# viniciusvidal2/slam-sensor-fusion

Hardware: AMD Instinct MI355X
Metric: scans_per_s_200k_scan_vs_10M_map (higher is better)
Workload: dtype f32 points / f64 accumulation

## Files before the change

### include/slamfusion.h

```cpp
#ifndef SLAMFUSION_H
#define SLAMFUSION_H
#include <stdint.h>

#ifdef __cplusplus
extern "C" {
#endif

#define SF_VERSION 210

typedef enum {
    SF_OK = 0,
    SF_ERR_INVALID = -1,
    SF_ERR_HIP = -2,
    SF_ERR_NOMEM = -3,
    SF_ERR_STATE = -4,
    SF_ERR_OVERFLOW = -5,
    SF_ERR_COMM = -6
} sf_status;

typedef struct sf_ctx sf_ctx;
typedef struct sf_cloud sf_cloud;
typedef struct sf_map sf_map;
typedef struct sf_icp sf_icp;

// ... 178 lines not shown
int sf_icp_fused_count(sf_icp *icp, int64_t *launches);
int sf_icp_fused_redone(sf_icp *icp, int64_t *redone);
int sf_icp_test_inject_barrier_timeout(sf_icp *icp);
#define SF_ORDER_AUTO 0
#define SF_ORDER_AS_GIVEN 1
#define SF_ORDER_CELL 2
int sf_icp_set_query_order(sf_icp *icp, int order);
int sf_icp_set_nn_reuse(sf_icp *icp, int on);
int sf_icp_set_wide_scan_points(sf_icp *icp, int64_t points);
int sf_icp_set_pipeline(sf_icp *icp, int on);
int sf_icp_set_tile_search(sf_icp *icp, int mode);
int sf_icp_tile_info(sf_icp *icp, int64_t out[12]);
int sf_icp_set_freeze(sf_icp *icp, int on);
int sf_icp_set_freeze_params(sf_icp *icp, float guard_scale, float guard_min, float guard_max, int max_tries, int from_launch);
int sf_icp_freeze_stats(sf_icp *icp, int64_t out[5]);
int sf_icp_set_defer_search(sf_icp *icp, int on);
int sf_icp_defer_stats(sf_icp *icp, int64_t out[2]);
int sf_icp_lookup_launch_stats(sf_icp *icp, int64_t out[4]);
int sf_icp_set_neighbour_research(sf_icp *icp, int from_launch);
int sf_icp_neighbour_stats(sf_icp *icp, int64_t out[3]);
int sf_icp_neighbour_gap_stats(sf_icp *icp, int64_t out[4]);
#define SF_ROBUST_NONE 0
#define SF_ROBUST_HUBER 1
#define SF_ROBUST_CAUCHY 2
#define SF_ROBUST_TUKEY 3
#define SF_ROBUST_GM 4
int sf_icp_set_robust_kernel(sf_icp *icp, int kind, double k);

#define SF_COV_EIG_EPS 1e-12
#define SF_COV_FEW_CORR 1
// ... 201 lines not shown
#define SF_TEST_OP_ROBUST 7
#define SF_TEST_OP_EIGVEC 8
int sf_test_linalg(sf_ctx *ctx, int op, const double *in, int in_stride, int64_t cases, double *out, int out_stride);
int sf_test_wave_reduce(sf_ctx *ctx, int width , const double *in , double *out );
int sf_test_block_reduce(sf_ctx *ctx, int nrec , const double *in , double *out );
int sf_test_reduce_partials(sf_ctx *ctx, int nrec , int nt , const double *part , int nblocks, double *out );

int sf_test_plane_score(sf_cloud *c, const float *planes, int64_t n_planes, double t, int max_blocks, int64_t *counts);

int sf_test_label_boxes(sf_cloud *c, const int32_t *labels, int64_t n_labels, const sf_box_params *p, int max_blocks,
                        sf_label_box *boxes, sf_box_stats *stats);

#define SF_TEST_SCHEDULE_IN 15
#define SF_TEST_SCHEDULE_OUT 10
int sf_test_launch_schedule(const int32_t *in, int64_t rows, int k, int32_t *out);

#ifdef __cplusplus
}
#endif
#endif
```

### slam_sensor_fusion_amd/api.py

```python
import atexit
import ctypes as C
import math
import os
import weakref

import numpy as np

_HERE = os.path.dirname(os.path.abspath(__file__))
LIB_PATH = os.path.join(_HERE, "lib", "libslamfusion.so")

SF_ICP_REF_CPP, SF_ICP_O3D_P2P, SF_ICP_P2PLANE = 0, 1, 2
SF_VOXEL_PCL, SF_VOXEL_O3D, SF_VOXEL_PCL64 = 0, 1, 2
SF_FLAG_VOXEL_OVERFLOW = 1
SF_ICP_FLAG_FEW_CORR, SF_ICP_FLAG_SINGULAR, SF_ICP_FLAG_SHARD_STALE, SF_ICP_FLAG_BARRIER_TIMEOUT = 1, 2, 4, 8
PROF_NN, PROF_REDUCE, PROF_COLLECTIVE, PROF_SOLVE, PROF_SHARD_BUILD = 0, 1, 2, 3, 4
SF_ERR_COMM = -6
MODES = {"ref_cpp": SF_ICP_REF_CPP, "o3d_p2p": SF_ICP_O3D_P2P, "p2plane": SF_ICP_P2PLANE}
ROBUST_KINDS = {"none": 0, "huber": 1, "cauchy": 2, "tukey": 3, "gm": 4}


class SlamFusionError(RuntimeError):
    pass


# ... 166 lines not shown
    lib.sf_test_linalg.argtypes = [C.c_void_p, C.c_int, C.c_void_p, C.c_int, C.c_int64, C.c_void_p, C.c_int]
    lib.sf_test_wave_reduce.argtypes = [C.c_void_p, C.c_int, C.c_void_p, C.c_void_p]
    lib.sf_test_block_reduce.argtypes = [C.c_void_p, C.c_int, C.c_void_p, C.c_void_p]
    lib.sf_test_reduce_partials.argtypes = [C.c_void_p, C.c_int, C.c_int, C.c_void_p, C.c_int, C.c_void_p]
    lib.sf_plane_default_params.restype = None
    lib.sf_cloud_plane_hypotheses.argtypes = [C.c_void_p, C.c_void_p, C.c_void_p, C.c_void_p, C.c_void_p]
    lib.sf_cloud_score_planes.argtypes = [C.c_void_p, C.c_void_p, C.c_int64, C.c_double, C.c_void_p]
    lib.sf_cloud_segment_plane.argtypes = [C.c_void_p, C.c_void_p, C.c_void_p, C.c_void_p, C.c_void_p]
    lib.sf_cloud_remove_plane.argtypes = [C.c_void_p, C.c_void_p, C.c_int, C.c_void_p, C.c_void_p]
    lib.sf_test_plane_score.argtypes = [C.c_void_p, C.c_void_p, C.c_int64, C.c_double, C.c_int, C.c_void_p]
    lib.sf_cloud_label_boxes.argtypes = [C.c_void_p, C.c_void_p, C.c_int64, C.c_void_p, C.c_void_p, C.c_void_p]
    lib.sf_test_label_boxes.argtypes = [C.c_void_p, C.c_void_p, C.c_int64, C.c_void_p, C.c_int, C.c_void_p, C.c_void_p]
    lib.sf_cloud_cluster_boxes.argtypes = [C.c_void_p, C.c_double, C.c_int64, C.c_int64, C.c_float, C.c_void_p, C.c_void_p, C.c_int64, C.c_void_p, C.c_void_p]
    lib.sf_cloud_remove_boxes.argtypes = [C.c_void_p, C.c_void_p, C.c_void_p, C.c_void_p, C.c_int64, C.c_double, C.c_int, C.c_void_p]
    lib.sf_test_launch_schedule.argtypes = [C.c_void_p, C.c_int64, C.c_int, C.c_void_p]
    _lib = lib
    return lib


def voxel_merge_min_points(n=-1):
    return int(load_library().sf_cloud_voxel_merge_min_points(C.c_int64(n)))


def kernel_source_hash():
    import hashlib
    h = hashlib.sha256()
    for name in ("sf_icp.hip", "sf_nn_red_body.inc", "sf_nn.hpp", "sf_tile.hpp", "sf_order.hpp", "sf_common.hpp", "sf_schedule.hpp"):
        with open(os.path.join(_HERE, "csrc", name), "rb") as f:
            h.update(f.read())
    return h.hexdigest()[:16]
# ... 14 lines not shown

def _p(a):
    return a.ctypes.data_as(C.c_void_p)


SCHEDULE_INPUTS = ("mode", "K", "qpl", "sharded", "whole", "reuse", "window", "robust", "wanted", "fz_from", "defer", "table", "nbr_from", "lk_min", "tile_on")
SCHEDULE_OUTPUTS = ("launches", "nn", "one_per_lane", "solve_takes_freeze_state", "ask_freeze", "deferred_rows", "attempt_from", "fz", "lookup_first", "defer_first")
NN_SEARCH, NN_TILE_SEARCH, NN_DEFERRING, NN_FREEZE, NN_FROZEN_FEW = range(5)


def hook_launch_schedule(configs, k):
    configs = np.ascontiguousarray(configs, dtype=np.int32).reshape(-1, len(SCHEDULE_INPUTS))
    out = np.empty((len(configs), len(SCHEDULE_OUTPUTS)), np.int32)
    _check(load_library().sf_test_launch_schedule(_p(configs), len(configs), int(k), _p(out)))
    return out


def hook_plane_score(cloud, planes, distance_threshold, max_blocks=0):
    planes = _f32(planes).reshape(-1, 4)
    counts = np.empty(len(planes), np.int64)
    _check(cloud.lib.sf_test_plane_score(cloud.h, _p(planes), len(planes), float(distance_threshold), int(max_blocks), _p(counts)))
    return counts


def hook_label_boxes(cloud, labels, n_labels=None, mode="pca", up=None, max_blocks=0):
    return cloud._label_boxes(labels, n_labels, mode, up, False, int(max_blocks))


def hook_radix_sort(ctx, keys, vals, end_bit, lead=0, lead_alt=0):
    keys = np.ascontiguousarray(keys)
# ... 698 lines not shown
        _check(self.lib.sf_icp_set_tile_search(self.h, C.c_int(code)))

    def tile_info(self):
        a = (C.c_int64 * 12)()
        _check(self.lib.sf_icp_tile_info(self.h, a))
        return {"on": bool(a[0]), "cells_per_tile": [a[1], a[2], a[3]], "tiles": [a[4], a[5], a[6]], "searched": a[7], "from_lds": a[8], "left_region": a[9],
                "beyond_ring_1": a[10], "tiles_too_dense": a[11]}

    def set_freeze_params(self, guard_scale=8.0, guard_min=2.0e-5, guard_max=3.0e-4, max_tries=3, from_launch=5):
        _check(self.lib.sf_icp_set_freeze_params(self.h, C.c_float(guard_scale), C.c_float(guard_min), C.c_float(guard_max), C.c_int(max_tries), C.c_int(from_launch)))

    def freeze_stats(self):
        a = (C.c_int64 * 5)()
        _check(self.lib.sf_icp_freeze_stats(self.h, a))
        return {"froze": a[0], "thawed": a[1], "failed": a[2], "active_queries": a[3], "frozen_at_end": a[4]}

    def set_defer_search(self, on=True):
        _check(self.lib.sf_icp_set_defer_search(self.h, C.c_int(int(bool(on)))))

    def set_neighbour_research(self, from_launch=2):
        _check(self.lib.sf_icp_set_neighbour_research(self.h, C.c_int(int(from_launch))))

    def neighbour_stats(self):
        a = (C.c_int64 * 3)()
        _check(self.lib.sf_icp_neighbour_stats(self.h, a))
        return {"served": a[0], "not_served": a[1], "waves_searched": a[2]}

    def neighbour_gap_stats(self):
        a = (C.c_int64 * 4)()
        _check(self.lib.sf_icp_neighbour_gap_stats(self.h, a))
# ... 674 lines not shown
```

### slam_sensor_fusion_amd/csrc/sf_icp.hip

```cpp
#include "sf_common.hpp"
#include "sf_nn.hpp"
#include "sf_tile.hpp"
#include "sf_order.hpp"
#include "sf_p2p.hpp"
#include "sf_schedule.hpp"

#include <cfloat>
#include <cstdlib>
#include <cmath>
#include <vector>
#include <mutex>
#include <string>

namespace {

constexpr int BLK = 256;
constexpr int NREC_P2P = 17;
constexpr int NREC_PLANE = 30;
constexpr int REC_STRIDE = 32;

struct IcpState {
    double T[16];
    double rec[REC_STRIDE];
    double fitness, rmse, prev_fitness, prev_rmse;
    float last_error, err_pending;
    float step[12];
    int step_pending;
    int iterations, done, research, n_corr, n_research, flags, converged;
    int n_points;
    int cache_live;
    int froze_launch;
    double T_list[12];
    double motion;
};

struct IcpParams {
    float max_corr;
    float accept;
    float eps;
    int num_iters;
};

inline unsigned nblk(int64_t n, int b = 256) { return (unsigned)sf::div_up(n > 0 ? n : 1, b); }

__device__ __forceinline__ void mat4_mul(const double A[16], const double B[16], double C[16])
{
    double R[16];
#pragma unroll
// ... 329 lines not shown
    int b = blockIdx.x * blockDim.x + threadIdx.x;
    if (b >= batch) return;
    IcpState s;
    for (int i = 0; i < 16; ++i) s.T[i] = inits ? inits[16 * b + i] : args.T[b][i];
    for (int i = 0; i < REC_STRIDE; ++i) s.rec[i] = 0;
    s.fitness = s.rmse = s.prev_fitness = s.prev_rmse = 0;
    s.last_error = FLT_MAX;
    s.err_pending = 0;
    for (int i = 0; i < 12; ++i) s.step[i] = 0;
    s.step_pending = 0;
    s.iterations = s.done = s.research = s.n_corr = s.n_research = s.flags = s.converged = 0;
    s.n_points = -1;
    s.cache_live = 0;
    s.froze_launch = -1;
    s.motion = 0.0;
    for (int i = 0; i < 12; ++i) s.T_list[i] = s.T[i];
    st[b] = s;
}

constexpr int64_t WIDE_SCAN_POINTS = 131072;
constexpr int64_t WIDE_AUTO_POINTS = 65536;
using sf::VERIFY_FROM_SEARCH;
#ifndef NN_RED_WAVES
#define NN_RED_WAVES 4
#endif
#ifndef SF_NBR_FROM
#define SF_NBR_FROM 2
#endif
constexpr int NN_STATS_SHARDS = 256;
constexpr int NN_STATS_PER = 5;
// ... 871 lines not shown

__device__ __forceinline__ void track_motion(IcpState *S, const double *To, const ScanBox &box)
{
    double worst = 0.0;
    for (int c = 0; c < 8; ++c) {
        const double x = (c & 1) ? box.hi[0] : box.lo[0], y = (c & 2) ? box.hi[1] : box.lo[1], z = (c & 4) ? box.hi[2] : box.lo[2];
        double d2 = 0.0;
        for (int r = 0; r < 3; ++r) {
            const double d = (S->T[4 * r] - To[4 * r]) * x + (S->T[4 * r + 1] - To[4 * r + 1]) * y + (S->T[4 * r + 2] - To[4 * r + 2]) * z + (S->T[4 * r + 3] - To[4 * r + 3]);
            d2 += d * d;
        }
        worst = d2 > worst ? d2 : worst;
    }
    const double step = sqrt(worst) * 1.000001 + 1.0e-9;
    S->motion = (step == step) ? S->motion + step : 1.0e30;
    S->cache_live = 1;
}

__device__ __forceinline__ void solve_o3d(IcpState *S, const double *rec, int n_src, int k, int K)
{
    k = S->n_research;
    const double n = rec[0];
    const double fitness = n_src > 0 ? n / (double)n_src : 0.0;
    const double rmse = n > 0 ? sqrt(rec[16] / n) : 0.0;
    S->fitness = fitness;
    S->rmse = rmse;
    S->n_corr = (int)n;
    S->n_research += 1;
    if (k > 0 && fabs(S->prev_fitness - fitness) < 1e-6 && fabs(S->prev_rmse - rmse) < 1e-6) {
        S->converged = 1;
// ... 76 lines not shown
constexpr int FZ_NMOM = 96;
constexpr int FZ_CAP = 128;
constexpr int64_t FREEZE_AUTO_MIN_QUERIES = 700000;
struct FreezeState {
    int mode;
    int tries;
    int froze, thawed;
    int64_t n_active;
    float guard;
    int launch_mode;
    double motion0;
    double Tf[12];
    double D[12];
    double mom[FZ_NMOM];
};
struct FreezeParams { float guard_scale, guard_min, guard_max; int max_tries; };

__device__ __forceinline__ constexpr int k6a(int k) { return k < 3 ? 0 : (k < 5 ? 1 : 2); }
__device__ __forceinline__ constexpr int k6b(int k) { return k < 3 ? k : (k < 5 ? k - 2 : 2); }
__device__ __forceinline__ constexpr int k6(int a, int b) { return a <= b ? (a == 0 ? b : (a == 1 ? 2 + b : 5)) : (b == 0 ? a : (b == 1 ? 2 + a : 5)); }

struct MomIn { double x[3], n[3], p[3], c, w; };
__device__ __forceinline__ MomIn mom_in(const LanePair &P, bool take)
{
    MomIn t;
    const bool ok = P.ok && take;
    t.w = ok ? 1.0 : 0.0;
    t.x[0] = ok ? P.sx : 0.0; t.x[1] = ok ? P.sy : 0.0; t.x[2] = ok ? P.sz : 0.0;
    t.p[0] = (double)(ok ? P.px : 0.0f); t.p[1] = (double)(ok ? P.py : 0.0f); t.p[2] = (double)(ok ? P.pz : 0.0f);
    t.n[0] = (double)(ok ? P.tn.x : 0.0f); t.n[1] = (double)(ok ? P.tn.y : 0.0f); t.n[2] = (double)(ok ? P.tn.z : 0.0f);
    t.c = t.n[0] * t.p[0] + t.n[1] * t.p[1] + t.n[2] * t.p[2];
// ... 654 lines not shown
                F->mode = 0;
                F->tries += 1;
            } else {
                F->mode = 2;
                F->froze += 1;
                if (S->froze_launch < 0) S->froze_launch = S->n_research;
                F->motion0 = S->motion;
                for (int i = 0; i < 12; ++i) { F->Tf[i] = S->T[i]; F->D[i] = (i % 5 == 0) ? 1.0 : 0.0; }
                for (int i = 0; i < FZ_NMOM; ++i) F->mom[i] = mom[i];
            }
        }
    }
    __syncthreads();
}

__device__ __forceinline__ void freeze_after_update(const IcpState *S, FreezeState *F, double m0, double m1, const FreezeParams &fp, int request, const double *upd)
{
    if (F->mode == 2) {
        double Dn[12];
        for (int r = 0; r < 3; ++r) {
            for (int c = 0; c < 4; ++c) Dn[4 * r + c] = upd[4 * r] * F->D[c] + upd[4 * r + 1] * F->D[4 + c] + upd[4 * r + 2] * F->D[8 + c] + (c == 3 ? upd[4 * r + 3] : 0.0);
        }
        for (int i = 0; i < 12; ++i) F->D[i] = Dn[i];
    }
    if (F->mode == 2 && !(m1 - F->motion0 <= (double)F->guard * 0.98)) {
        F->mode = 0;
        F->tries += 1;
        F->thawed += 1;
    }
    if (F->mode == 0 && F->launch_mode == 0 && request && !S->done && F->tries < fp.max_tries) {
        const float gd = fmaxf((float)(m1 - m0) * fp.guard_scale, fp.guard_min);
        if (gd <= fp.guard_max) { F->guard = gd; F->mode = 1; }
    }
}

__global__ __launch_bounds__(RBLK) void k_reduce_solve_fz(IcpState *__restrict__ st, const double *__restrict__ partials, int nblocks, int n_src, int K,
                                                          const ScanBox *__restrict__ boxp, FreezeBufs fb, FreezeParams fp, int request)
{
    const int b = blockIdx.x;
    IcpState *S = st + b;
    if (S->done) return;
    FreezeState *F = fb.fz + b;
    __shared__ double rec[REC_STRIDE];
    freeze_fold<RBLK>(S, F, b, partials, nblocks, nblocks, fb, rec);
    if (fb.df_part) add_deferred_rows(fb.df_part, b, rec);
    if (threadIdx.x == 0) {
        for (int c = 0; c < NREC_PLANE; ++c) S->rec[c] = rec[c];
        double To[12];
// ... 579 lines not shown
    int64_t fused_redone = 0;
    bool inject_timeout = false;
    int64_t fused_launches = 0;
    IcpState *h_pin = nullptr;
    size_t h_pin_cap = 0;
    bool use_graph = false;
    int64_t graph_captures = 0, graph_replays = 0;
    struct GraphKey {
        int batch = -1, ordered = -1, robust_kind = -1, cov_on = -1;
        sf::Schedule sched;
        int64_t n = -1;
        const void *map = nullptr;
        uint64_t map_generation = 0, epochs = 0;
        uint64_t nbr_stamp = 0;
        const void *nbr = nullptr;
        float max_corr = 0, accept = 0, eps = 0, guard_scale = 0, guard_min = 0, guard_max = 0;
        int max_tries = 0;
        double robust_k = 0;
        double cov_prm[5] = {0, 0, 0, 0, 0};
        bool operator==(const GraphKey &o) const
        {
            return batch == o.batch && ordered == o.ordered && sched == o.sched && n == o.n && map == o.map && map_generation == o.map_generation && epochs == o.epochs &&
                   nbr_stamp == o.nbr_stamp && nbr == o.nbr && max_corr == o.max_corr && accept == o.accept && eps == o.eps &&
                   guard_scale == o.guard_scale && guard_min == o.guard_min && guard_max == o.guard_max && max_tries == o.max_tries &&
                   robust_kind == o.robust_kind && robust_k == o.robust_k && cov_on == o.cov_on && std::memcmp(cov_prm, o.cov_prm, sizeof(cov_prm)) == 0;
        }
    };
    struct LaneMeta {
        bool valid = false;
        bool cov = false;
        int batch = 0, mode = 0;
        std::vector<double> inits;
        int src_set = 0;
        uint64_t src_version = 0;
        sf::Schedule sched;
        int64_t lk_waves = 0;
    };
    struct Lane {
        sf::DevBuf X;
// ... 55 lines not shown
    bool unfetched = false;
    bool mark_valid = false;
    uint64_t src_version = 0, mark_src_version = 0, mark_map_generation = 0;
    const void *mark_map = nullptr;
    SfWindow mark_window{};
    bool profiling = false;
    std::vector<hipEvent_t> ev;
    size_t ev_used = 0;
    int64_t prof_launches = 0;
    double prof_ms = 0;
    std::vector<float> prof_each;
    std::vector<int> ev_kind;
    std::vector<float> prof_phase[SF_PROF_KINDS];
    sf::DevBuf nn_stats;
    int freeze = 1;
    FreezeParams fz_prm{8.0f, 2.0e-5f, 3.0e-4f, 3};
    int fz_from = 5;
    bool fz_from_auto = true;
    int fz_fetches = 0;
    int fz_step = 0;
    int nbr_from = SF_NBR_FROM;
    bool nbr_active = false;
    int64_t nbr_stats_first = 0;
    uint64_t mark_nbr_stamp = 0;
    int defer = 1;
    int lk_min = 0;
    int64_t nn_stats_used = 0;
    static constexpr int64_t NN_STATS_CAP = 1024;
    int robust_kind = SF_ROBUST_NONE;
    double robust_k = 0.0;
    int cov_on = 0;
    CovArg cov_arg{0.0, 0.0, 0.0, 0.0, 0.0};
    bool prev_cov_ok = false;
    int tile_mode = 0;
// ... 392 lines not shown
}

sf_icp::GraphKey graph_key_now(const sf_icp *icp, int mode)
{
    const Lane &ln = icp->cur(); const SrcSet &ss = icp->src();
    sf_icp::GraphKey k;
    k.batch = ss.batch; k.ordered = (int)icp->ordered; k.sched = ln.meta.sched;
    k.n = (mode == SF_ICP_REF_CPP && ss.batch == 1) ? -ss.n_cap : ss.n;
    k.map = (const void *)icp->map;
    k.map_generation = icp->map->generation;
    if (icp->nbr_active) { k.nbr_stamp = icp->map->nbr_stamp; k.nbr = icp->map->nbr.p; }
    k.robust_kind = robust_on(icp, mode) ? icp->robust_kind : SF_ROBUST_NONE; k.robust_k = robust_on(icp, mode) ? icp->robust_k : 0.0;
    k.cov_on = icp->cov_on;
    if (icp->cov_on) { const double cp[5] = {icp->cov_arg.sensor_sigma, icp->cov_arg.thr_t, icp->cov_arg.thr_r, icp->cov_arg.infl_t, icp->cov_arg.infl_r}; std::memcpy(k.cov_prm, cp, sizeof(cp)); }
    k.max_corr = icp->prm.max_corr; k.accept = icp->prm.accept; k.eps = icp->prm.eps;
    k.guard_scale = icp->fz_prm.guard_scale; k.guard_min = icp->fz_prm.guard_min; k.guard_max = icp->fz_prm.guard_max; k.max_tries = icp->fz_prm.max_tries;
    const sf::DevBuf *bufs[] = {&ss.X0, &ss.X0r, &ln.X, &ln.Xq, &ln.qcache, &ln.corr, &ln.state, &ln.partials, &icp->d_box, &ss.d_boxes, &ss.n_dev,
                                &icp->map->pts4, &icp->map->nrm4, &icp->map->cell_start, &icp->map->d_window, &ln.fz_state, &ln.fz_part, &ln.fz_cnt, &ln.fz_ids, &ln.fz_all, &ln.df_cnt, &ln.df_ids, &ln.df_part, &ln.df_stat, &ln.tseg, &ln.tile_stats, &ln.cov_part, &ln.cov_out};
    k.epochs = (uint64_t)ss.plane;
    for (const sf::DevBuf *b : bufs) k.epochs = (k.epochs * 1000003ull + b->epoch) * 1000003ull + (uint64_t)(uintptr_t)b->p;
    return k;
}

SfGrid grid_for(const sf_icp *icp)
{
    SfGrid g = icp->map->grid;
    g.nbr = icp->nbr_active ? icp->map->nbr.as<uint4>() : nullptr;
    g.nbr_from = icp->nbr_from;
    return g;
}

// ... 841 lines not shown
    out[1] = df[0];
    out[2] = df[1];
    out[3] = sched.lookup_first;
    return SF_OK;
}

extern "C" int sf_icp_set_freeze(sf_icp *icp, int on)
{
    SF_CHECK(icp, SF_ERR_INVALID, "icp is NULL");
    SF_CHECK(on >= 0 && on <= 2, SF_ERR_INVALID, "sf_icp_set_freeze: 0 (off), 1 (auto) or 2 (always)");
    icp->freeze = on;
    return SF_OK;
}

namespace {
constexpr int FZ_FROM_DEFAULT = 5, FZ_PROBE_EVERY = 32;
void freeze_learn_schedule(sf_icp *icp)
{
    const sf::Schedule &sched = icp->cur().meta.sched;
    if (!icp->fz_from_auto || icp->last_fused || icp->shard || icp->last_mode != SF_ICP_P2PLANE) return;
    const int K = sched.K;
    if (++icp->fz_fetches >= FZ_PROBE_EVERY) { icp->fz_fetches = 0; icp->fz_from = FZ_FROM_DEFAULT; icp->lk_min = 0; return; }
    if (!sched.fz) return;
    if (sched.lookup_launches() > 0 && icp->cur().df_stat.p) {
        uint32_t h[2 + DF_STAT_LAUNCHES];
        if (hipMemcpy(h, icp->cur().df_stat.p, sizeof(h), hipMemcpyDeviceToHost) == hipSuccess) {
            for (int k = sched.lookup_first; k < sched.fz_from && k < DF_STAT_LAUNCHES - 1; ++k)
                if ((int64_t)h[2 + k] * 8 > icp->cur().meta.lk_waves) icp->lk_min = std::max(icp->lk_min, k + 1);
        }
    }
    int latest = -1, never = 0;
    for (int b = 0; b < icp->src().batch; ++b) {
        const IcpState &S = icp->h_state[(size_t)b];
        if (S.froze_launch >= 0) latest = std::max(latest, S.froze_launch);
        else if (S.iterations >= K) never += 1;
    }
    if (latest < 0) icp->fz_from = std::max(FZ_FROM_DEFAULT, K);
    else if (never * 4 <= icp->src().batch) icp->fz_from = std::min(std::max(FZ_FROM_DEFAULT, latest), std::max(FZ_FROM_DEFAULT, K - 2));
}
}

extern "C" int sf_icp_set_robust_kernel(sf_icp *icp, int kind, double k)
{
    SF_CHECK(icp, SF_ERR_INVALID, "icp is NULL");
    SF_CHECK(kind >= SF_ROBUST_NONE && kind <= SF_ROBUST_GM, SF_ERR_INVALID, "unknown robust kernel %d", kind);
    SF_CHECK(kind == SF_ROBUST_NONE || (std::isfinite(k) && k > 0.0), SF_ERR_INVALID, "the robust kernel's scale must be finite and > 0 (got %g)", k);
    icp->robust_kind = kind;
    icp->robust_k = kind == SF_ROBUST_NONE ? 0.0 : k;
    return SF_OK;
}

extern "C" int sf_icp_set_freeze_params(sf_icp *icp, float guard_scale, float guard_min, float guard_max, int max_tries, int from_launch)
{
    SF_CHECK(icp, SF_ERR_INVALID, "icp is NULL");
    SF_CHECK(guard_scale >= 0.0f && guard_min >= 0.0f && guard_max >= guard_min && max_tries >= 0 && from_launch >= VERIFY_FROM_SEARCH && from_launch < 1024, SF_ERR_INVALID,
             "bad freeze parameters");
    icp->fz_prm = FreezeParams{guard_scale, guard_min, guard_max, max_tries};
    icp->fz_from = from_launch;
    icp->fz_from_auto = false;
    icp->lk_min = 0;
    return SF_OK;
}

extern "C" int sf_icp_freeze_stats(sf_icp *icp, int64_t out[5])
{
    SF_CHECK(icp && out, SF_ERR_INVALID, "bad arguments");
    Lane &ln = icp->cur(); SrcSet &ss = icp->src();
    for (int i = 0; i < 5; ++i) out[i] = 0;
    const int nb = ln.meta.valid && ln.meta.batch > 0 && !icp->shard ? ln.meta.batch : ss.batch;
    if (!ln.meta.sched.fz || icp->last_fused || !ln.fz_state.p || nb <= 0) return SF_OK;
    std::vector<FreezeState> h((size_t)nb);
    SF_HIP(hipMemcpyAsync(h.data(), ln.fz_state.p, sizeof(FreezeState) * h.size(), hipMemcpyDeviceToHost, icp->ctx->stream));
    SF_HIP(hipStreamSynchronize(icp->ctx->stream));
    for (const FreezeState &f : h) {
        out[0] += f.froze;
        out[1] += f.thawed;
        out[2] += f.tries - f.thawed;
        out[3] += f.n_active;
        out[4] += f.mode == 2 ? 1 : 0;
    }
    return SF_OK;
}

extern "C" int sf_icp_graph_counts(sf_icp *icp, int64_t *captures, int64_t *launches)
{
    SF_CHECK(icp, SF_ERR_INVALID, "icp is NULL");
    if (captures) *captures = icp->graph_captures;
    if (launches) *launches = icp->graph_replays;
    return SF_OK;
}

extern "C" int sf_icp_set_fused(sf_icp *icp, int on)
{
    SF_CHECK(icp, SF_ERR_INVALID, "icp is NULL");
    icp->fused = on != 0;
// ... 236 lines not shown

extern "C" int sf_icp_fetch_results(sf_icp *icp, sf_icp_result *out)
{
    SF_CHECK(icp && out, SF_ERR_INVALID, "bad arguments");
    const Lane &ln = icp->cur(); const SrcSet &ss = icp->src();
    SF_CHECK(ss.batch > 0, SF_ERR_STATE, "nothing to fetch");
    const bool described = ln.meta.valid && ln.meta.batch > 0 && !icp->shard;
    const int nb = described ? ln.meta.batch : ss.batch;
    SF_TRY(states_to_host(icp, nb));
    icp->unfetched = false;
    fused_release(icp);
    if (icp->profiling) prof_collect(icp);
    SF_TRY(check_barrier_flags(icp, nb));
    for (int b = 0; b < nb; ++b)
        fill_result(icp, described ? ln.meta.mode : icp->last_mode, icp->h_state[(size_t)b], described ? &ln.meta.inits[(size_t)b * 16] : &icp->inits[(size_t)b * 16], out + b);
    if (nb == ss.batch) freeze_learn_schedule(icp);
    return SF_OK;
}

extern "C" int sf_icp_fetch_previous(sf_icp *icp, sf_icp_result *out)
{
    SF_CHECK(icp && out, SF_ERR_INVALID, "bad arguments");
    Lane &pl = icp->prev();
    const sf_icp::LaneMeta &M = pl.meta;
    SF_CHECK(icp->prev_ok && M.valid && M.batch > 0, SF_ERR_STATE,
             "no earlier alignment to fetch: the latest alignment did not run beside the one before it (fetched in between, pipeline off, single launch) or it was fetched already");
    SF_CHECK(pl.used && pl.done && pl.stream && pl.state.p, SF_ERR_STATE, "the other lane holds no alignment");
    SF_HIP(hipSetDevice(icp->ctx->device));
    SF_HIP(hipEventSynchronize(pl.done));
    icp->h_prev.resize((size_t)M.batch);
    SF_HIP(hipMemcpyAsync(icp->h_prev.data(), pl.state.p, sizeof(IcpState) * (size_t)M.batch, hipMemcpyDeviceToHost, pl.stream));
    SF_HIP(hipStreamSynchronize(pl.stream));
    for (int b = 0; b < M.batch; ++b) fill_result(icp, M.mode, icp->h_prev[(size_t)b], &M.inits[(size_t)b * 16], out + b);
    icp->prev_ok = false;
    return SF_OK;
}

extern "C" int sf_icp_set_covariance(sf_icp *icp, int on, double sensor_sigma)
{
    SF_CHECK(icp, SF_ERR_INVALID, "icp is NULL");
    SF_CHECK(std::isfinite(sensor_sigma) && sensor_sigma >= 0.0, SF_ERR_INVALID, "sensor_sigma must be finite and >= 0 (0: the estimated residual variance)");
    icp->cov_on = on != 0;
    icp->cov_arg.sensor_sigma = sensor_sigma;
    return SF_OK;
}

extern "C" int sf_icp_set_degeneracy_thresholds(sf_icp *icp, double trans, double rot, double inflate_trans_var, double inflate_rot_var)
{
    SF_CHECK(icp, SF_ERR_INVALID, "icp is NULL");
// ... 470 lines not shown
```

### slam_sensor_fusion_amd/csrc/sf_schedule.hpp

```cpp
#pragma once
#include "slamfusion.h"

#ifndef SF_WIDE_QPL
#define SF_WIDE_QPL 2
#endif

namespace sf {

constexpr int VERIFY_FROM_SEARCH = 4;

struct Schedule {
    int mode = 0, K = 0, qpl = 1;
    int sharded = 0, whole = 0;
    int reuse = 0, window = 0;
    int robust = 0, wanted = 0;
    int fz_from = 0, defer = 0;
    int table = 0, nbr_from = 0;
    int lk_min = 0, tile_on = 0;
    int fz = 0, lookup_first = 0, defer_first = 0;
    bool operator==(const Schedule &o) const
    {
        return mode == o.mode && K == o.K && qpl == o.qpl && sharded == o.sharded && whole == o.whole && reuse == o.reuse && window == o.window && robust == o.robust &&
               wanted == o.wanted && fz_from == o.fz_from && defer == o.defer && table == o.table && nbr_from == o.nbr_from && lk_min == o.lk_min && tile_on == o.tile_on &&
               fz == o.fz && lookup_first == o.lookup_first && defer_first == o.defer_first;
// ... 31 lines not shown
{
    LaunchStep st;
    const bool df = k >= s.defer_first && k < s.fz_from;
    st.one_per_lane = s.mode == SF_ICP_P2PLANE && s.qpl > 1 && k < VERIFY_FROM_SEARCH && !df;
    if (s.fz && k == s.fz_from) st.nn = NN_FREEZE;
    else if (s.fz && k > s.fz_from) st.nn = NN_FROZEN_FEW;
    else if (df) st.nn = NN_DEFERRING;
    else if (s.whole && s.tile_on && (!s.reuse || k < VERIFY_FROM_SEARCH)) st.nn = NN_TILE_SEARCH;
    st.solve_takes_freeze_state = s.fz && k + 1 >= s.fz_from;
    st.ask_freeze = st.solve_takes_freeze_state && k + 2 < s.K;
    st.deferred_rows = df;
    st.attempt_from = s.lookup_first < s.fz_from ? s.lookup_first : VERIFY_FROM_SEARCH;
    return st;
}

}
```

### slam_sensor_fusion_amd/csrc/sf_testhooks.hip

```cpp
#include "sf_common.hpp"

#include "sf_sort.hpp"
#include "sf_schedule.hpp"

namespace {

constexpr int64_t GUARD = 4096;
constexpr int64_t TEST_MAX_N = (int64_t)1 << 26;
constexpr int GUARD_BYTE = 0xA5;
constexpr uint32_t GUARD_WORD = 0xA5A5A5A5u;

struct Carve {
    size_t off = 0, elem = 0;
    int64_t lead = 0, n = 0;
    size_t front_bytes() const { return (size_t)(GUARD + lead) * elem; }
    size_t data_off() const { return off + front_bytes(); }
    size_t data_bytes() const { return (size_t)n * elem; }
    size_t back_off() const { return data_off() + data_bytes(); }
    size_t back_bytes() const { return (size_t)GUARD * elem; }
    size_t end() const { return (back_off() + back_bytes() + 15u) & ~(size_t)15u; }
};

Carve carve_after(size_t off, size_t elem, int64_t lead, int64_t n)
{
// ... 72 lines not shown
    SF_CHECK(rows >= 0, SF_ERR_INVALID, "sf_test_launch_schedule: rows %lld < 0", (long long)rows);
    for (int64_t r = 0; r < rows; ++r) {
        const int32_t *v = in + r * SF_TEST_SCHEDULE_IN;
        sf::Schedule s;
        s.mode = v[0]; s.K = v[1]; s.qpl = v[2]; s.sharded = v[3]; s.whole = v[4]; s.reuse = v[5]; s.window = v[6]; s.robust = v[7]; s.wanted = v[8]; s.fz_from = v[9];
        s.defer = v[10]; s.table = v[11]; s.nbr_from = v[12]; s.lk_min = v[13]; s.tile_on = v[14];
        s = sf::make_schedule(s);
        const sf::LaunchStep st = sf::step_of(s, k);
        const int32_t o[SF_TEST_SCHEDULE_OUT] = {sf::launches(s), st.nn, st.one_per_lane, st.solve_takes_freeze_state, st.ask_freeze, st.deferred_rows, st.attempt_from,
                                                 s.fz, s.lookup_first, s.defer_first};
        std::memcpy(out + r * SF_TEST_SCHEDULE_OUT, o, sizeof(o));
    }
    return SF_OK;
}

extern "C" int sf_test_scan_u32(sf_ctx *ctx, int op, const uint32_t *in, int64_t n, uint32_t carry0, int in_place, uint32_t *out, int64_t *guard_damage)
{
    SF_CHECK(ctx && guard_damage, SF_ERR_INVALID, "sf_test_scan_u32: ctx or guard_damage is NULL");
    SF_CHECK(op == 0 || op == 1, SF_ERR_INVALID, "sf_test_scan_u32: op %d (0: exclusive sum, 1: inclusive max)", op);
    SF_CHECK(n >= 0 && n <= TEST_MAX_N, SF_ERR_INVALID, "sf_test_scan_u32: n %lld outside [0, 2^26]", (long long)n);
    SF_CHECK((in && out) || n == 0, SF_ERR_INVALID, "sf_test_scan_u32: in or out is NULL");
    SF_HIP(hipSetDevice(ctx->device));
    Carve a[2];
    a[0] = carve_after(0, sizeof(uint32_t), 0, n);
    a[1] = carve_after(a[0].end(), sizeof(uint32_t), 0, n);
    const int narr = in_place ? 1 : 2;
    const size_t total = a[narr - 1].end();
    sf::DevBuf buf;
    SF_TRY(buf.reserve(total));
    char *base = buf.as<char>();
// ... 17 lines not shown
```

Measured before the change: 22210.

## Learn an earlier freeze launch with a motion-based guard for ICP

Each scan now records its accumulated motion at the early search launches, and the host-side freeze learner moves into a testable schedule header. When earlier alignments froze cleanly at the default launch, the learner can schedule freezing one launch earlier, with a guard derived from the remaining motion. This skips nearest-neighbour search launches. If freezing fails, thaws, or leaves many active queries, it backs off to the later launch. Learning now also runs on the pipelined fetch path, which adds a small device-to-host copy and stream sync there. The cost is extra per-state fields and the risk that an early freeze misjudges correspondences.

```diff
diff --git a/include/slamfusion.h b/include/slamfusion.h
--- a/include/slamfusion.h
+++ b/include/slamfusion.h
@@ -216,6 +216,8 @@
 int sf_icp_set_freeze(sf_icp *icp, int on);
 int sf_icp_set_freeze_params(sf_icp *icp, float guard_scale, float guard_min, float guard_max, int max_tries, int from_launch);
 int sf_icp_freeze_stats(sf_icp *icp, int64_t out[5]);
+int sf_icp_freeze_schedule(sf_icp *icp, int64_t out[4], double *early_guard);
+int sf_icp_froze_launches(sf_icp *icp, int previous, int32_t *out, int64_t count);
 int sf_icp_set_defer_search(sf_icp *icp, int on);
 int sf_icp_defer_stats(sf_icp *icp, int64_t out[2]);
 int sf_icp_lookup_launch_stats(sf_icp *icp, int64_t out[4]);
@@ -447,6 +449,10 @@
 #define SF_TEST_SCHEDULE_IN 15
 #define SF_TEST_SCHEDULE_OUT 10
 int sf_test_launch_schedule(const int32_t *in, int64_t rows, int k, int32_t *out);
+#define SF_TEST_LEARN_IN 11
+#define SF_TEST_LEARN_IN_D 3
+#define SF_TEST_LEARN_MARKS 2
+int sf_test_freeze_learn(const int64_t *in_i, const double *in_d, int64_t rows, int scans, int64_t *out_i, double *out_d);
 
 #ifdef __cplusplus
 }
diff --git a/slam_sensor_fusion_amd/api.py b/slam_sensor_fusion_amd/api.py
--- a/slam_sensor_fusion_amd/api.py
+++ b/slam_sensor_fusion_amd/api.py
@@ -204,6 +204,9 @@
     lib.sf_cloud_cluster_boxes.argtypes = [C.c_void_p, C.c_double, C.c_int64, C.c_int64, C.c_float, C.c_void_p, C.c_void_p, C.c_int64, C.c_void_p, C.c_void_p]
     lib.sf_cloud_remove_boxes.argtypes = [C.c_void_p, C.c_void_p, C.c_void_p, C.c_void_p, C.c_int64, C.c_double, C.c_int, C.c_void_p]
     lib.sf_test_launch_schedule.argtypes = [C.c_void_p, C.c_int64, C.c_int, C.c_void_p]
+    lib.sf_test_freeze_learn.argtypes = [C.c_void_p, C.c_void_p, C.c_int64, C.c_int, C.c_void_p, C.c_void_p]
+    lib.sf_icp_freeze_schedule.argtypes = [C.c_void_p, C.c_void_p, C.c_void_p]
+    lib.sf_icp_froze_launches.argtypes = [C.c_void_p, C.c_int, C.c_void_p, C.c_int64]
     _lib = lib
     return lib
 
@@ -248,6 +251,21 @@
     out = np.empty((len(configs), len(SCHEDULE_OUTPUTS)), np.int32)
     _check(load_library().sf_test_launch_schedule(_p(configs), len(configs), int(k), _p(out)))
     return out
+
+
+LEARN_STATE = ("fz_from", "lk_min", "fetches", "early_off")
+LEARN_INPUTS = LEARN_STATE + ("automatic", "fz", "ran_fz_from", "K", "seen_lk_min", "queries", "lookup_first")
+LEARN_SCAN = ("froze_launch", "iterations", "tries", "thawed", "active")
+LEARN_MARKS = 2
+
+
+def hook_freeze_learn(ints, floats, scans):
+    ints = np.ascontiguousarray(ints, dtype=np.int64).reshape(-1, len(LEARN_INPUTS) + len(LEARN_SCAN) * scans)
+    floats = np.ascontiguousarray(floats, dtype=np.float64).reshape(-1, 3 + (1 + LEARN_MARKS) * scans)
+    assert len(ints) == len(floats)
+    out_i, out_d = np.empty((len(ints), len(LEARN_STATE)), np.int64), np.empty(len(ints), np.float64)
+    _check(load_library().sf_test_freeze_learn(_p(ints), _p(floats), len(ints), int(scans), _p(out_i), _p(out_d)))
+    return out_i, out_d
 
 
 def hook_plane_score(cloud, planes, distance_threshold, max_blocks=0):
@@ -976,6 +994,17 @@
         a = (C.c_int64 * 5)()
         _check(self.lib.sf_icp_freeze_stats(self.h, a))
         return {"froze": a[0], "thawed": a[1], "failed": a[2], "active_queries": a[3], "frozen_at_end": a[4]}
+
+    def freeze_schedule(self):
+        a, g = (C.c_int64 * 4)(), C.c_double()
+        _check(self.lib.sf_icp_freeze_schedule(self.h, a, C.byref(g)))
+        return {"from_launch": a[0], "automatic": bool(a[1]), "early_off": bool(a[2]), "fetches": a[3], "early_guard": g.value}
+
+    def froze_launches(self, previous=False, batch=None):
+        n = int(batch or getattr(self, "_prev_batch" if previous else "_last_batch", None) or self.batch)
+        out = np.empty(n, np.int32)
+        _check(self.lib.sf_icp_froze_launches(self.h, C.c_int(int(bool(previous))), _p(out), n))
+        return out.tolist()
 
     def set_defer_search(self, on=True):
         _check(self.lib.sf_icp_set_defer_search(self.h, C.c_int(int(bool(on)))))
diff --git a/slam_sensor_fusion_amd/csrc/sf_icp.hip b/slam_sensor_fusion_amd/csrc/sf_icp.hip
--- a/slam_sensor_fusion_amd/csrc/sf_icp.hip
+++ b/slam_sensor_fusion_amd/csrc/sf_icp.hip
@@ -32,6 +32,8 @@
     int froze_launch;
     double T_list[12];
     double motion;
+    double motion_mark[sf::MOTION_MARKS];
+    int fz_tries, fz_thawed, fz_active;
 };
 
 struct IcpParams {
@@ -391,6 +393,8 @@
     s.cache_live = 0;
     s.froze_launch = -1;
     s.motion = 0.0;
+    for (int i = 0; i < sf::MOTION_MARKS; ++i) s.motion_mark[i] = -1.0;
+    s.fz_tries = s.fz_thawed = s.fz_active = 0;
     for (int i = 0; i < 12; ++i) s.T_list[i] = s.T[i];
     st[b] = s;
 }
@@ -1292,6 +1296,8 @@
     }
     const double step = sqrt(worst) * 1.000001 + 1.0e-9;
     S->motion = (step == step) ? S->motion + step : 1.0e30;
+    const int mark = S->n_research - VERIFY_FROM_SEARCH;
+    if (mark >= 0 && mark < sf::MOTION_MARKS) S->motion_mark[mark] = S->motion;
     S->cache_live = 1;
 }
 
@@ -1398,7 +1404,11 @@
     double D[12];
     double mom[FZ_NMOM];
 };
-struct FreezeParams { float guard_scale, guard_min, guard_max; int max_tries; };
+struct FreezeParams {
+    float guard_scale, guard_min, guard_max;
+    int max_tries;
+    float early_guard;
+};
 
 __device__ __forceinline__ constexpr int k6a(int k) { return k < 3 ? 0 : (k < 5 ? 1 : 2); }
 __device__ __forceinline__ constexpr int k6b(int k) { return k < 3 ? k : (k < 5 ? k - 2 : 2); }
@@ -2083,7 +2093,7 @@
     __syncthreads();
 }
 
-__device__ __forceinline__ void freeze_after_update(const IcpState *S, FreezeState *F, double m0, double m1, const FreezeParams &fp, int request, const double *upd)
+__device__ __forceinline__ void freeze_after_update(IcpState *S, FreezeState *F, double m0, double m1, const FreezeParams &fp, int request, const double *upd)
 {
     if (F->mode == 2) {
         double Dn[12];
@@ -2098,9 +2108,11 @@
         F->thawed += 1;
     }
     if (F->mode == 0 && F->launch_mode == 0 && request && !S->done && F->tries < fp.max_tries) {
-        const float gd = fmaxf((float)(m1 - m0) * fp.guard_scale, fp.guard_min);
-        if (gd <= fp.guard_max) { F->guard = gd; F->mode = 1; }
-    }
+        const bool early = S->n_research < sf::FZ_FROM_DEFAULT && fp.early_guard > 0.0f;
+        const float gd = early ? fp.early_guard : fmaxf((float)(m1 - m0) * fp.guard_scale, fp.guard_min);
+        if (early || gd <= fp.guard_max) { F->guard = gd; F->mode = 1; }
+    }
+    S->fz_tries = F->tries; S->fz_thawed = F->thawed; S->fz_active = (int)F->n_active;
 }
 
 __global__ __launch_bounds__(RBLK) void k_reduce_solve_fz(IcpState *__restrict__ st, const double *__restrict__ partials, int nblocks, int n_src, int K,
@@ -2710,7 +2722,7 @@
         uint64_t map_generation = 0, epochs = 0;
         uint64_t nbr_stamp = 0;
         const void *nbr = nullptr;
-        float max_corr = 0, accept = 0, eps = 0, guard_scale = 0, guard_min = 0, guard_max = 0;
+        float max_corr = 0, accept = 0, eps = 0, guard_scale = 0, guard_min = 0, guard_max = 0, early_guard = 0;
         int max_tries = 0;
         double robust_k = 0;
         double cov_prm[5] = {0, 0, 0, 0, 0};
@@ -2718,7 +2730,7 @@
         {
             return batch == o.batch && ordered == o.ordered && sched == o.sched && n == o.n && map == o.map && map_generation == o.map_generation && epochs == o.epochs &&
                    nbr_stamp == o.nbr_stamp && nbr == o.nbr && max_corr == o.max_corr && accept == o.accept && eps == o.eps &&
-                   guard_scale == o.guard_scale && guard_min == o.guard_min && guard_max == o.guard_max && max_tries == o.max_tries &&
+                   guard_scale == o.guard_scale && guard_min == o.guard_min && guard_max == o.guard_max && early_guard == o.early_guard && max_tries == o.max_tries &&
                    robust_kind == o.robust_kind && robust_k == o.robust_k && cov_on == o.cov_on && std::memcmp(cov_prm, o.cov_prm, sizeof(cov_prm)) == 0;
         }
     };
@@ -2804,10 +2816,11 @@
     std::vector<float> prof_phase[SF_PROF_KINDS];
     sf::DevBuf nn_stats;
     int freeze = 1;
-    FreezeParams fz_prm{8.0f, 2.0e-5f, 3.0e-4f, 3};
-    int fz_from = 5;
+    FreezeParams fz_prm{8.0f, 2.0e-5f, 3.0e-4f, 3, 0.0f};
+    int fz_from = sf::FZ_FROM_DEFAULT;
     bool fz_from_auto = true;
     int fz_fetches = 0;
+    int fz_early_off = 0;
     int fz_step = 0;
     int nbr_from = SF_NBR_FROM;
     bool nbr_active = false;
@@ -3230,7 +3243,7 @@
     k.cov_on = icp->cov_on;
     if (icp->cov_on) { const double cp[5] = {icp->cov_arg.sensor_sigma, icp->cov_arg.thr_t, icp->cov_arg.thr_r, icp->cov_arg.infl_t, icp->cov_arg.infl_r}; std::memcpy(k.cov_prm, cp, sizeof(cp)); }
     k.max_corr = icp->prm.max_corr; k.accept = icp->prm.accept; k.eps = icp->prm.eps;
-    k.guard_scale = icp->fz_prm.guard_scale; k.guard_min = icp->fz_prm.guard_min; k.guard_max = icp->fz_prm.guard_max; k.max_tries = icp->fz_prm.max_tries;
+    k.guard_scale = icp->fz_prm.guard_scale; k.guard_min = icp->fz_prm.guard_min; k.guard_max = icp->fz_prm.guard_max; k.early_guard = icp->fz_prm.early_guard; k.max_tries = icp->fz_prm.max_tries;
     const sf::DevBuf *bufs[] = {&ss.X0, &ss.X0r, &ln.X, &ln.Xq, &ln.qcache, &ln.corr, &ln.state, &ln.partials, &icp->d_box, &ss.d_boxes, &ss.n_dev,
                                 &icp->map->pts4, &icp->map->nrm4, &icp->map->cell_start, &icp->map->d_window, &ln.fz_state, &ln.fz_part, &ln.fz_cnt, &ln.fz_ids, &ln.fz_all, &ln.df_cnt, &ln.df_ids, &ln.df_part, &ln.df_stat, &ln.tseg, &ln.tile_stats, &ln.cov_part, &ln.cov_out};
     k.epochs = (uint64_t)ss.plane;
@@ -4102,29 +4115,33 @@
 }
 
 namespace {
-constexpr int FZ_FROM_DEFAULT = 5, FZ_PROBE_EVERY = 32;
-void freeze_learn_schedule(sf_icp *icp)
-{
-    const sf::Schedule &sched = icp->cur().meta.sched;
-    if (!icp->fz_from_auto || icp->last_fused || icp->shard || icp->last_mode != SF_ICP_P2PLANE) return;
-    const int K = sched.K;
-    if (++icp->fz_fetches >= FZ_PROBE_EVERY) { icp->fz_fetches = 0; icp->fz_from = FZ_FROM_DEFAULT; icp->lk_min = 0; return; }
-    if (!sched.fz) return;
-    if (sched.lookup_launches() > 0 && icp->cur().df_stat.p) {
+void freeze_learn_schedule(sf_icp *icp, const Lane &ln, const IcpState *states, int mode, hipStream_t stream)
+{
+    const sf::Schedule &sched = ln.meta.sched;
+    if (!icp->fz_from_auto || icp->shard || mode != SF_ICP_P2PLANE) return;
+    sf::FetchedAlignment a;
+    a.fz = sched.fz; a.fz_from = sched.fz_from; a.K = sched.K; a.batch = ln.meta.batch; a.queries = ln.meta.lk_waves * 64 * sched.qpl; a.lookup_first = sched.lookup_first;
+    if (sched.fz && icp->fz_fetches + 1 < sf::FZ_PROBE_EVERY && sched.lookup_launches() > 0 && ln.df_stat.p) {
         uint32_t h[2 + DF_STAT_LAUNCHES];
-        if (hipMemcpy(h, icp->cur().df_stat.p, sizeof(h), hipMemcpyDeviceToHost) == hipSuccess) {
+        hipError_t e = stream ? hipMemcpyAsync(h, ln.df_stat.p, sizeof(h), hipMemcpyDeviceToHost, stream) : hipMemcpy(h, ln.df_stat.p, sizeof(h), hipMemcpyDeviceToHost);
+        if (e == hipSuccess && stream) e = hipStreamSynchronize(stream);
+        if (e == hipSuccess) {
             for (int k = sched.lookup_first; k < sched.fz_from && k < DF_STAT_LAUNCHES - 1; ++k)
-                if ((int64_t)h[2 + k] * 8 > icp->cur().meta.lk_waves) icp->lk_min = std::max(icp->lk_min, k + 1);
-        }
-    }
-    int latest = -1, never = 0;
-    for (int b = 0; b < icp->src().batch; ++b) {
-        const IcpState &S = icp->h_state[(size_t)b];
-        if (S.froze_launch >= 0) latest = std::max(latest, S.froze_launch);
-        else if (S.iterations >= K) never += 1;
-    }
-    if (latest < 0) icp->fz_from = std::max(FZ_FROM_DEFAULT, K);
-    else if (never * 4 <= icp->src().batch) icp->fz_from = std::min(std::max(FZ_FROM_DEFAULT, latest), std::max(FZ_FROM_DEFAULT, K - 2));
+                if ((int64_t)h[2 + k] * 8 > ln.meta.lk_waves) a.lk_min = std::max(a.lk_min, k + 1);
+        }
+    }
+    std::vector<sf::FetchedScan> scans((size_t)std::max(a.batch, 0));
+    for (int b = 0; b < a.batch; ++b) {
+        const IcpState &S = states[b];
+        sf::FetchedScan &f = scans[(size_t)b];
+        f.froze_launch = S.froze_launch; f.iterations = S.iterations; f.tries = S.fz_tries; f.thawed = S.fz_thawed; f.active = S.fz_active; f.motion = S.motion;
+        for (int i = 0; i < sf::MOTION_MARKS; ++i) f.mark[i] = S.motion_mark[i];
+    }
+    a.scans = scans.data();
+    sf::FreezeLearnt now;
+    now.fz_from = icp->fz_from; now.lk_min = icp->lk_min; now.fetches = icp->fz_fetches; now.early_off = icp->fz_early_off; now.early_guard = icp->fz_prm.early_guard;
+    now = sf::freeze_learn(now, 1, a, icp->fz_prm.guard_min, icp->fz_prm.guard_max);
+    icp->fz_from = now.fz_from; icp->lk_min = now.lk_min; icp->fz_fetches = now.fetches; icp->fz_early_off = now.early_off; icp->fz_prm.early_guard = now.early_guard;
 }
 }
 
@@ -4143,10 +4160,11 @@
     SF_CHECK(icp, SF_ERR_INVALID, "icp is NULL");
     SF_CHECK(guard_scale >= 0.0f && guard_min >= 0.0f && guard_max >= guard_min && max_tries >= 0 && from_launch >= VERIFY_FROM_SEARCH && from_launch < 1024, SF_ERR_INVALID,
              "bad freeze parameters");
-    icp->fz_prm = FreezeParams{guard_scale, guard_min, guard_max, max_tries};
+    icp->fz_prm = FreezeParams{guard_scale, guard_min, guard_max, max_tries, 0.0f};
     icp->fz_from = from_launch;
     icp->fz_from_auto = false;
     icp->lk_min = 0;
+    icp->fz_early_off = 0;
     return SF_OK;
 }
 
@@ -4167,6 +4185,23 @@
         out[3] += f.n_active;
         out[4] += f.mode == 2 ? 1 : 0;
     }
+    return SF_OK;
+}
+
+extern "C" int sf_icp_freeze_schedule(sf_icp *icp, int64_t out[4], double *early_guard)
+{
+    SF_CHECK(icp && out, SF_ERR_INVALID, "bad arguments");
+    out[0] = icp->fz_from; out[1] = icp->fz_from_auto ? 1 : 0; out[2] = icp->fz_early_off; out[3] = icp->fz_fetches;
+    if (early_guard) *early_guard = (double)icp->fz_prm.early_guard;
+    return SF_OK;
+}
+
+extern "C" int sf_icp_froze_launches(sf_icp *icp, int previous, int32_t *out, int64_t count)
+{
+    SF_CHECK(icp && out && count >= 0, SF_ERR_INVALID, "bad arguments");
+    const std::vector<IcpState> &h = previous ? icp->h_prev : icp->h_state;
+    SF_CHECK((size_t)count <= h.size(), SF_ERR_STATE, "sf_icp_froze_launches: %lld scans asked for, %lld fetched", (long long)count, (long long)h.size());
+    for (int64_t b = 0; b < count; ++b) out[b] = h[(size_t)b].froze_launch;
     return SF_OK;
 }
 
@@ -4433,7 +4468,7 @@
     SF_TRY(check_barrier_flags(icp, nb));
     for (int b = 0; b < nb; ++b)
         fill_result(icp, described ? ln.meta.mode : icp->last_mode, icp->h_state[(size_t)b], described ? &ln.meta.inits[(size_t)b * 16] : &icp->inits[(size_t)b * 16], out + b);
-    if (nb == ss.batch) freeze_learn_schedule(icp);
+    if (nb == ss.batch && !icp->last_fused) freeze_learn_schedule(icp, ln, icp->h_state.data(), icp->last_mode, nullptr);
     return SF_OK;
 }
 
@@ -4452,6 +4487,7 @@
     SF_HIP(hipStreamSynchronize(pl.stream));
     for (int b = 0; b < M.batch; ++b) fill_result(icp, M.mode, icp->h_prev[(size_t)b], &M.inits[(size_t)b * 16], out + b);
     icp->prev_ok = false;
+    freeze_learn_schedule(icp, pl, icp->h_prev.data(), M.mode, pl.stream);
     return SF_OK;
 }
 
diff --git a/slam_sensor_fusion_amd/csrc/sf_schedule.hpp b/slam_sensor_fusion_amd/csrc/sf_schedule.hpp
--- a/slam_sensor_fusion_amd/csrc/sf_schedule.hpp
+++ b/slam_sensor_fusion_amd/csrc/sf_schedule.hpp
@@ -69,4 +69,82 @@
     return st;
 }
 
+constexpr int FZ_FROM_DEFAULT = 5, FZ_PROBE_EVERY = 32;
+constexpr int MOTION_MARKS = FZ_FROM_DEFAULT - VERIFY_FROM_SEARCH + 1;
+#ifndef SF_EARLY_GUARD_FACTOR
+#define SF_EARLY_GUARD_FACTOR 2.0f
+#endif
+constexpr float EARLY_GUARD_FACTOR = SF_EARLY_GUARD_FACTOR;
+constexpr int EARLY_ACTIVE_DEN = 256;
+constexpr long long EARLY_MIN_QUERIES = 4000000;
+
+struct FreezeLearnt {
+    int fz_from = FZ_FROM_DEFAULT;
+    int lk_min = 0;
+    int fetches = 0;
+    int early_off = 0;
+    float early_guard = 0.0f;
+};
+struct FetchedScan {
+    int froze_launch = -1, iterations = 0, tries = 0, thawed = 0, active = 0;
+    double motion = 0.0;
+    double mark[MOTION_MARKS] = {};
+};
+struct FetchedAlignment {
+    int fz = 0, fz_from = 0, K = 0, batch = 0;
+    int lk_min = 0;
+    int lookup_first = 0;
+    long long queries = 0;
+    const FetchedScan *scans = nullptr;
+};
+
+inline FreezeLearnt freeze_learn(FreezeLearnt now, int automatic, const FetchedAlignment &a, float guard_min, float guard_max)
+{
+    if (!automatic) return now;
+    if (++now.fetches >= FZ_PROBE_EVERY) {
+        now.fetches = 0;
+        now.lk_min = 0;
+        if (now.fz_from >= FZ_FROM_DEFAULT || now.early_off) { now.fz_from = FZ_FROM_DEFAULT; now.early_off = 0; now.early_guard = 0.0f; }
+        return now;
+    }
+    if (!a.fz) return now;
+    if (a.lk_min > now.lk_min) now.lk_min = a.lk_min;
+    int latest = -1, never = 0, live = 0, at_first = 0, thawed = 0, failed = 0;
+    long long active = 0;
+    for (int b = 0; b < a.batch; ++b) {
+        const FetchedScan &s = a.scans[b];
+        thawed += s.thawed;
+        failed += s.tries - s.thawed;
+        active += s.active;
+        if (s.froze_launch >= 0) { latest = s.froze_launch > latest ? s.froze_launch : latest; live += 1; at_first += s.froze_launch == a.fz_from; }
+        else if (s.iterations >= a.K) { never += 1; live += 1; }
+    }
+    const bool clean = live > 0 && at_first == live && thawed == 0 && failed == 0;
+    if (a.fz_from < FZ_FROM_DEFAULT) {
+        if (now.fz_from != a.fz_from) return now;
+        if (!clean || active * EARLY_ACTIVE_DEN > a.queries) { now.fz_from = a.fz_from + 1; now.early_off = 1; now.early_guard = 0.0f; }
+        return now;
+    }
+    if (now.fz_from < FZ_FROM_DEFAULT) return now;
+    const int far = FZ_FROM_DEFAULT > a.K - 2 ? FZ_FROM_DEFAULT : a.K - 2;
+    if (latest < 0) now.fz_from = FZ_FROM_DEFAULT > a.K ? FZ_FROM_DEFAULT : a.K;
+    else if (never * 4 <= a.batch) now.fz_from = latest < FZ_FROM_DEFAULT ? FZ_FROM_DEFAULT : (latest < far ? latest : far);
+    const int early = FZ_FROM_DEFAULT - 1;
+    if (a.fz_from == FZ_FROM_DEFAULT && now.fz_from == FZ_FROM_DEFAULT && clean && !now.early_off && early >= VERIFY_FROM_SEARCH && a.K > early + 1 && a.lookup_first < early &&
+        a.queries >= EARLY_MIN_QUERIES) {
+        double left = 0.0;
+        bool known = true;
+        for (int b = 0; b < a.batch; ++b) {
+            const FetchedScan &s = a.scans[b];
+            if (s.froze_launch < 0) continue;
+            const double m = s.mark[early - VERIFY_FROM_SEARCH];
+            if (!(m >= 0.0) || !(s.motion >= m)) { known = false; break; }
+            left = s.motion - m > left ? s.motion - m : left;
+        }
+        const float g = (float)(left * (double)EARLY_GUARD_FACTOR) > guard_min ? (float)(left * (double)EARLY_GUARD_FACTOR) : guard_min;
+        if (known && g <= guard_max) { now.fz_from = early; now.early_guard = g; }
+    }
+    return now;
 }
+
+}
diff --git a/slam_sensor_fusion_amd/csrc/sf_testhooks.hip b/slam_sensor_fusion_amd/csrc/sf_testhooks.hip
--- a/slam_sensor_fusion_amd/csrc/sf_testhooks.hip
+++ b/slam_sensor_fusion_amd/csrc/sf_testhooks.hip
@@ -110,6 +110,35 @@
     return SF_OK;
 }
 
+extern "C" int sf_test_freeze_learn(const int64_t *in_i, const double *in_d, int64_t rows, int scans, int64_t *out_i, double *out_d)
+{
+    static_assert(SF_TEST_LEARN_MARKS == sf::MOTION_MARKS, "the hook passes every motion mark");
+    SF_CHECK((in_i && in_d && out_i && out_d) || rows == 0, SF_ERR_INVALID, "sf_test_freeze_learn: an array is NULL");
+    SF_CHECK(rows >= 0 && scans >= 0 && scans <= 4096, SF_ERR_INVALID, "sf_test_freeze_learn: rows %lld < 0 or scans %d outside [0, 4096]", (long long)rows, scans);
+    std::vector<sf::FetchedScan> sc((size_t)scans);
+    for (int64_t r = 0; r < rows; ++r) {
+        const int64_t *v = in_i + r * (SF_TEST_LEARN_IN + 5 * (int64_t)scans);
+        const double *d = in_d + r * (SF_TEST_LEARN_IN_D + (1 + SF_TEST_LEARN_MARKS) * (int64_t)scans);
+        sf::FreezeLearnt now;
+        now.fz_from = (int)v[0]; now.lk_min = (int)v[1]; now.fetches = (int)v[2]; now.early_off = (int)v[3]; now.early_guard = (float)d[0];
+        sf::FetchedAlignment a;
+        a.fz = (int)v[5]; a.fz_from = (int)v[6]; a.K = (int)v[7]; a.lk_min = (int)v[8]; a.queries = v[9]; a.lookup_first = (int)v[10]; a.batch = scans;
+        for (int b = 0; b < scans; ++b) {
+            const int64_t *s = v + SF_TEST_LEARN_IN + 5 * b;
+            const double *m = d + SF_TEST_LEARN_IN_D + (1 + SF_TEST_LEARN_MARKS) * b;
+            sf::FetchedScan &f = sc[(size_t)b];
+            f.froze_launch = (int)s[0]; f.iterations = (int)s[1]; f.tries = (int)s[2]; f.thawed = (int)s[3]; f.active = (int)s[4];
+            f.motion = m[0];
+            for (int i = 0; i < SF_TEST_LEARN_MARKS; ++i) f.mark[i] = m[1 + i];
+        }
+        a.scans = sc.data();
+        now = sf::freeze_learn(now, (int)v[4], a, (float)d[1], (float)d[2]);
+        out_i[4 * r] = now.fz_from; out_i[4 * r + 1] = now.lk_min; out_i[4 * r + 2] = now.fetches; out_i[4 * r + 3] = now.early_off;
+        out_d[r] = (double)now.early_guard;
+    }
+    return SF_OK;
+}
+
 extern "C" int sf_test_scan_u32(sf_ctx *ctx, int op, const uint32_t *in, int64_t n, uint32_t carry0, int in_place, uint32_t *out, int64_t *guard_damage)
 {
     SF_CHECK(ctx && guard_damage, SF_ERR_INVALID, "sf_test_scan_u32: ctx or guard_damage is NULL");
```

New measurement: 21940. 0.988x the previous value.
